# HarrisonKramer/optiland

Hardware: AMD Instinct MI355X
Metric: ray-surface intersections/s (higher is better)
Workload: dtype f32

## Files before the change

### include/optiland_hip.h

```cpp
#ifndef OPTILAND_HIP_H
#define OPTILAND_HIP_H

#include <stdint.h>

#ifdef __cplusplus
extern "C" {
#endif

#define OL_ABI_VERSION 11

#define OL_OK 0
#define OL_EINVAL (-1)
#define OL_EUNSUPPORTED (-2)
#define OL_EHIP (-3)
#define OL_ENOMEM (-4)

typedef int32_t ol_dtype;
enum { OL_F32 = 0, OL_F64 = 1 };

typedef enum ol_geom_kind {
  OL_GEOM_PLANE = 0,
  OL_GEOM_STANDARD = 1,
  OL_GEOM_EVEN_ASPHERE = 2,
  OL_GEOM_ZERNIKE = 3,
// ... 292 lines not shown
                   double Rp, double* psf_out, double* field_out, void* stream);

#define OL_MTF_MAX_CURVES 64
#define OL_MTF_MAX_BINS 8192
#define OL_MTF_NONFINITE 1
int ol_geometric_mtf(ol_dtype dt, int32_t n_curves, const void* const* coords,
                     const int64_t* lengths, int32_t num_points, const double* freq,
                     const double* scale, int32_t n_bins, double* mtf_out, int32_t* counts_out,
                     double* edges_minmax_out, int32_t* flags_out, void* stream);

#define OL_ZK_MAX_TERMS 120
#define OL_ZK_MAX_RADIAL 12
#define OL_ZK_MAX_M 32
#define OL_ZK_TOO_FEW 1
#define OL_ZK_RANK_DEFICIENT 2
#define OL_ZK_NONFINITE 4
#define OL_SMTF_MAX_FREQ 65535
int ol_zernike_fit(int32_t num_terms, const int32_t* term_i, const double* term_f, int64_t n,
                   const double* x, const double* y, const double* z, const double* intensity,
                   double* coeffs_out, int32_t* status_out, void* stream);
int ol_zernike_eval(int32_t num_terms, const int32_t* term_i, const double* term_f,
                    const double* coeffs, int64_t n, const double* x, const double* y,
                    double* out, void* stream);
int ol_sampled_mtf(int32_t num_terms, const int32_t* term_i, const double* term_f,
                   const double* coeffs, int64_t n, const double* x, const double* y,
                   const double* opd_waves, const double* p1, const double* intensity,
                   int32_t n_freq, const double* shifts, double* mtf_out, double* otf_out,
                   void* stream);

#define OL_TUNE_RAYS_PER_THREAD 0
#define OL_TUNE_COMPACT 1
#define OL_TUNE_FIT_GRID 2
#define OL_TUNE_RECORD_WG_CAP 3
int ol_set_tuning(int32_t knob, int32_t value);

const char* ol_last_error(void);
int32_t ol_abi_version(void);

#ifdef __cplusplus
}
#endif
#endif
```

### optiland_amd/_capi.py

```python

from __future__ import annotations

import ctypes as C
import os

from . import build as _build

_LIB = None


class HipExtensionError(RuntimeError):
    """The HIP shared library is missing / failed to load / returned an error."""


class SurfaceDesc(C.Structure):
    _fields_ = [
        ("geom_kind", C.c_int32),
        ("interaction", C.c_int32),
        ("aperture_kind", C.c_int32),
        ("coating_kind", C.c_int32),
        ("coeff_offset", C.c_int32),
        ("n_coeff", C.c_int32),
        ("max_iter", C.c_int32),
        ("flags", C.c_uint32),
# ... 85 lines not shown
    "ol_system_destroy",
    "ol_system_num_surfaces",
    "ol_trace",
    "ol_generate_rays",
    "ol_polarized_intensity",
    "ol_spot_moments",
    "ol_spot_max_r2",
    "ol_set_tuning",
    "ol_wavefront_opd",
    "ol_trace_spot",
    "ol_trace_ex",
    "ol_radial_energy",
    "ol_irradiance",
    "ol_trace_opd",
    "ol_pupil_fill",
    "ol_trace_generate",
    "ol_system_update",
    "ol_stream_fill",
    "ol_math_probe",
    "ol_pupil_points",
    "ol_wavefront_reference",
    "ol_trace_opd_dev",
    "ol_wavefront_fit",
    "ol_wavefront_opd_fitted",
    "ol_trace_spot_batch",
    "ol_newton_count",
    "ol_arena_alloc",
    "ol_arena_free",
    "ol_huygens_psf",
    "ol_geometric_mtf",
    "ol_zernike_fit",
    "ol_zernike_eval",
    "ol_sampled_mtf",
)

F32, F64 = 0, 1
TUNE_RAYS_PER_THREAD, TUNE_COMPACT, TUNE_FIT_GRID, TUNE_RECORD_WG_CAP = 0, 1, 2, 3
ABI_VERSION = 11
OPD_MOMENTS = 12
WAVEFRONT_REFERENCE_DOUBLES = 16
WAVEFRONT_FIT_WORKSPACE_DOUBLES = 32832
FIT_CENTROID, FIT_BEST_FIT = 0, 1
FIT_NO_VALID, FIT_TOO_FEW, FIT_NO_ALIVE, FIT_SINGULAR = 1, 2, 4, 8
FIT_STD_DDOF1, FIT_PISTON_SKIPS_NAN = 1, 2


def library_path() -> str:
    return os.environ.get("OPTILAND_HIP_LIBRARY", _build.library_path())


def load():
    global _LIB
    if _LIB is not None:
        return _LIB
    path = library_path()
    if not os.path.exists(path):
        raise HipExtensionError(
            f"HIP extension not built: {path} is missing. Run "
            "`python -c 'import __graft_entry__ as g; g.build()'` (needs hipcc). "
            "optiland_amd has no CPU fallback."
        )
    try:
        lib = C.CDLL(path)
    except OSError as exc:
        raise HipExtensionError(f"cannot load {path}: {exc}") from exc
    if hasattr(lib, "ol_hostmath_harness"):
        raise HipExtensionError(f"{path} is the host-math TEST harness, not the HIP extension")
    bind(lib, path)
    _LIB = lib
    return lib
# ... 49 lines not shown
        raise HipExtensionError(
            f"{path}: ABI version {have} != expected {ABI_VERSION}; rebuild"
        )
    lib.ol_wavefront_reference.restype = C.c_int
    lib.ol_wavefront_reference.argtypes = [vp, i32, vp, vp, vp, C.c_double, i32, i32, vp, vp, vp,
                                           vp]
    lib.ol_trace_opd_dev.restype = C.c_int
    lib.ol_trace_opd_dev.argtypes = [vp, i32, i64, vp, vp, vp, i32, vp, vp, C.POINTER(vp), vp,
                                     vp, vp]
    lib.ol_wavefront_fit.restype = C.c_int
    lib.ol_wavefront_fit.argtypes = [i32, vp, C.c_double, C.c_uint32, i32, i64, C.POINTER(vp), vp, vp,
                                     vp, vp, vp, vp]
    lib.ol_wavefront_opd_fitted.restype = C.c_int
    lib.ol_wavefront_opd_fitted.argtypes = [i64, C.POINTER(vp), vp, vp, vp, vp, C.POINTER(vp), vp]
    lib.ol_system_update.restype = C.c_int
    lib.ol_system_update.argtypes = [vp, vp, i32, vp, i32, vp, i32, vp]
    lib.ol_trace_generate.restype = C.c_int
    lib.ol_trace_generate.argtypes = [vp, C.c_int, i64, vp, vp, i32, vp, i64, C.POINTER(vp), vp,
                                      u32, vp, vp, vp]
    lib.ol_trace_spot_batch.restype = C.c_int
    lib.ol_trace_spot_batch.argtypes = [vp, C.c_int, i64, vp, vp, i32, vp, vp, i64, vp, vp, vp]
    lib.ol_newton_count.restype = C.c_int
    lib.ol_newton_count.argtypes = [vp, C.c_int, i64, C.POINTER(vp), i32, i32, i32, vp, i32, vp]
    lib.ol_arena_alloc.restype = C.c_int
    lib.ol_arena_alloc.argtypes = [i64, C.POINTER(vp)]
    lib.ol_arena_free.restype = C.c_int
    lib.ol_arena_free.argtypes = [vp]
    lib.ol_pupil_points.restype = C.c_int
    lib.ol_pupil_points.argtypes = [i32, i32, C.c_int, i64, vp, vp, vp, vp, vp]
    lib.ol_math_probe.restype = C.c_int
    lib.ol_math_probe.argtypes = [i32, C.c_int, i64, vp, vp, vp, vp]
    lib.ol_stream_fill.restype = C.c_int
    lib.ol_stream_fill.argtypes = [vp, i64, i32, i32, u32, vp]
    if hasattr(lib, "ol_huygens_psf"):
        lib.ol_huygens_psf.restype = C.c_int
        lib.ol_huygens_psf.argtypes = [i64, C.POINTER(vp), vp, i64, C.POINTER(vp), C.c_double,
                                       C.c_double, vp, vp, vp]
    if hasattr(lib, "ol_geometric_mtf"):
        lib.ol_geometric_mtf.restype = C.c_int
        lib.ol_geometric_mtf.argtypes = [C.c_int, i32, C.POINTER(vp), C.POINTER(i64), i32, vp, vp,
                                         i32, vp, vp, vp, vp, vp]
    if has_zernike_fit(lib):
        lib.ol_zernike_fit.restype = C.c_int
        lib.ol_zernike_fit.argtypes = [i32, vp, vp, i64, vp, vp, vp, vp, vp, vp, vp]
        lib.ol_zernike_eval.restype = C.c_int
        lib.ol_zernike_eval.argtypes = [i32, vp, vp, vp, i64, vp, vp, vp, vp]
        lib.ol_sampled_mtf.restype = C.c_int
        lib.ol_sampled_mtf.argtypes = [i32, vp, vp, vp, i64, vp, vp, vp, vp, vp, i32, vp, vp, vp,
                                       vp]
    return lib


ZK_MAX_TERMS, ZK_MAX_RADIAL, ZK_MAX_M, SMTF_MAX_FREQ = 120, 12, 32, 65535
ZK_TOO_FEW, ZK_RANK_DEFICIENT, ZK_NONFINITE = 1, 2, 4


def has_zernike_fit(lib) -> bool:
    return all(hasattr(lib, s) for s in ("ol_zernike_fit", "ol_zernike_eval", "ol_sampled_mtf"))


MTF_MAX_CURVES, MTF_MAX_BINS, MTF_NONFINITE = 64, 8192, 1


def has_geometric_mtf(lib) -> bool:
    return hasattr(lib, "ol_geometric_mtf")

# ... 12 lines not shown
```

### optiland_amd/csrc/capi.hip

```cpp
#include <hip/hip_runtime.h>

#include <algorithm>
#include <cmath>
#include <cstdarg>
#include <cstdio>
#include <cstdlib>
#include <cstring>
#include <map>
#include <new>
#include <string>
#include <type_traits>
#include <vector>

#include "../../include/optiland_hip.h"
#include "device_table.h"
#include "last_error.h"
#include "trace_launch.h"

namespace {
thread_local std::string g_err;
}

int ol::failf(int code, const char* fmt, ...) {
  char buf[512];
// ... 150 lines not shown
        }
      }
    }
  }
  for (int i = nmax; i >= 0; --i)
    for (int j = nmax - i; j >= 0; --j) out.push_back(S[i * W + j]);
  for (int i = nmax - 1; i >= 0; --i)
    for (int j = nmax - 1 - i; j >= 0; --j) {
      out.push_back((i + 1) * Q[(i + 1) * W + j]);
      out.push_back((j + 1) * Q[i * W + j + 1]);
    }
  *degree = nmax;
  return true;
}

struct HostSurf {
  int32_t geom, interaction, aperture_kind, coating_kind, coeff_off, n_coeff, max_iter;
  uint32_t flags;
  int32_t poly_cols, coeff_len, ap_off, ap_len;
  double cv, kp1, tol, inv_norm;
  double origin[3], rot[9], rel_off[3], rel_rot[9], ap[4], coat[2], axis[3], ret_cos, ret_sin;
  double radius, conic;
};

template <typename T>
struct DeviceTable {
  char* blob = nullptr;
  ol::DevSurfHot<T>* surf = nullptr;
  ol::DevSurfCold<T>* cold = nullptr;
  ol::DevOptics<T>* optics = nullptr;
  T* coeffs = nullptr;
  size_t n_surf = 0, n_opt = 0, coef_capacity = 0;
  size_t off_cold = 0, off_opt = 0, off_coef = 0;
};

inline size_t round256(size_t v) { return (v + 255u) & ~size_t(255u); }

struct Staged {
  std::vector<struct HostSurf> surf;
  std::vector<ol::DevOptics<double>> optics;
  std::vector<double> coeffs;
  std::vector<size_t> int_slots;
  std::vector<int32_t> interaction, coating, geom;
  std::vector<uint8_t> polygon, ref_newton, no_pair;
};

}

struct ol_system {
  int32_t n_surf = 0;
  int32_t n_wl = 0;
  int device = 0;
  DeviceTable<float> f32;
  DeviceTable<double> f64;
  std::vector<int32_t> interaction;
  std::vector<int32_t> coating;
  std::vector<int32_t> geom;
  std::vector<uint8_t> polygon;
  std::vector<uint8_t> ref_newton;
  std::vector<uint8_t> no_pair;
  bool consistent = true;
};

#define OL_CHECK_CONSISTENT(sys, who)                                                          \
  if (!(sys)->consistent)                                                                      \
    return failf(OL_EINVAL, who ": the system's tables are inconsistent after a failed "         \
                                "ol_system_update (destroy it and create a new one)")

namespace {

template <typename T>
int upload(const std::vector<HostSurf>& surf64,
           const std::vector<ol::DevOptics<double>>& opt64, const std::vector<double>& coef64,
           const std::vector<size_t>& int_slots, DeviceTable<T>& dst, bool in_place = false,
           hipStream_t stream = nullptr) {
  const size_t n_surf = surf64.size(), n_opt = opt64.size();
  const size_t n_coef = coef64.size() ? coef64.size() : 1;
  const size_t off_cold = round256(n_surf * sizeof(ol::DevSurfHot<T>));
  const size_t off_opt = off_cold + round256(n_surf * sizeof(ol::DevSurfCold<T>));
  const size_t off_coef = off_opt + round256(n_opt * sizeof(ol::DevOptics<T>));
  const size_t used = off_coef + n_coef * sizeof(T);
  std::vector<char> host(used, 0);
  auto* surf = reinterpret_cast<ol::DevSurfHot<T>*>(host.data());
  auto* cold = reinterpret_cast<ol::DevSurfCold<T>*>(host.data() + off_cold);
  auto* opt = reinterpret_cast<ol::DevOptics<T>*>(host.data() + off_opt);
  T* coef = reinterpret_cast<T*>(host.data() + off_coef);
  for (size_t i = 0; i < n_surf; ++i) {
    const auto& a = surf64[i];
    auto& b = surf[i];
    auto& c = cold[i];
    b.geom = a.geom; b.interaction = a.interaction; b.aperture_kind = a.aperture_kind;
    b.coating_kind = a.coating_kind; b.coeff_off = a.coeff_off; b.n_coeff = a.n_coeff;
    b.max_iter = a.max_iter; b.flags = a.flags;
    b.cv = (T)a.cv; b.kp1 = (T)a.kp1;
    c.poly_cols = a.poly_cols; c.coeff_len = a.coeff_len; c.ap_off = a.ap_off;
    c.ap_len = a.ap_len; c.tol = (T)a.tol; c.inv_norm = (T)a.inv_norm;
    for (int k = 0; k < 3; ++k) { b.origin[k] = (T)a.origin[k]; b.rel_off[k] = (T)a.rel_off[k]; }
    for (int k = 0; k < 9; ++k) { c.rot[k] = (T)a.rot[k]; c.rel_rot[k] = (T)a.rel_rot[k]; }
    for (int k = 0; k < 4; ++k) c.ap[k] = (T)a.ap[k];
    for (int k = 0; k < 2; ++k) c.coat[k] = (T)a.coat[k];
    for (int k = 0; k < 3; ++k) c.axis[k] = (T)a.axis[k];
    c.ret_cos = (T)a.ret_cos; c.ret_sin = (T)a.ret_sin;
    c.radius = (T)a.radius; c.conic = (T)a.conic;
  }
  for (size_t i = 0; i < n_opt; ++i) {
    opt[i].n1 = (T)opt64[i].n1; opt[i].n2 = (T)opt64[i].n2; opt[i].u = (T)opt64[i].u;
    opt[i].nn = (T)opt64[i].nn; opt[i].absorb = (T)opt64[i].absorb;
  }
  for (size_t i = 0; i < coef64.size(); ++i) coef[i] = (T)coef64[i];
  for (size_t i : int_slots) {
    using I = typename std::conditional<sizeof(T) == 4, int32_t, int64_t>::type;
    const I v = (I)coef64[i];
    std::memcpy(&coef[i], &v, sizeof(T));
  }

  if (in_place) {
    OL_HIP_CHECK(hipMemcpyAsync(dst.blob, host.data(), used, hipMemcpyHostToDevice, stream));
    return OL_OK;
  }
  dst.n_surf = n_surf;
  dst.n_opt = n_opt;
  dst.coef_capacity = n_coef + 64;
  dst.off_cold = off_cold; dst.off_opt = off_opt; dst.off_coef = off_coef;
  OL_HIP_CHECK(hipMalloc((void**)&dst.blob, off_coef + dst.coef_capacity * sizeof(T)));
  dst.surf = reinterpret_cast<ol::DevSurfHot<T>*>(dst.blob);
  dst.cold = reinterpret_cast<ol::DevSurfCold<T>*>(dst.blob + off_cold);
  dst.optics = reinterpret_cast<ol::DevOptics<T>*>(dst.blob + off_opt);
  dst.coeffs = reinterpret_cast<T*>(dst.blob + off_coef);
  OL_HIP_CHECK(hipMemcpy(dst.blob, host.data(), used, hipMemcpyHostToDevice));
  return OL_OK;
}

template <typename T>
void release(DeviceTable<T>& t) {
  if (t.blob) (void)hipFree(t.blob);
  t = DeviceTable<T>();
}

bool aligned16(const void* p) { return (reinterpret_cast<uintptr_t>(p) & 15u) == 0; }

int newton_family(const ol_system* sys, int32_t first, int32_t last) {
  bool any = false, polygon = false, all_zernike = true, all_even = true;
  for (int32_t s = first; s <= last; ++s)
    if (sys->ref_newton[s]) return ol::kNrReference;
  for (int32_t s = first; s <= last; ++s) {
    polygon = polygon || sys->polygon[s];
    const int g = sys->geom[s];
    if (g == OL_GEOM_PLANE || g == OL_GEOM_STANDARD) continue;
// ... 148 lines not shown
  if (a.in.hx == nullptr) ol::uniform_field_tangents<T>(rg, a.in);
  for (int k = 0; k < 8; ++k) a.rays[k] = rays_out ? static_cast<T*>(rays_out[k]) : nullptr;
  a.record = static_cast<T*>(record);
  a.prt = static_cast<T*>(prt);
  a.status = status;
  a.n = n;
  a.record_stride = record_stride;
  a.first = 0;
  a.last = sys->n_surf - 1;
  a.record_from = (extras && extras->record_first_surface > 0) ? extras->record_first_surface : 0;
  a.n_wl = sys->n_wl;
  a.wl = wl;
  a.flags = (flags & (ol::kTracePrtComplex | ol::kTraceFewWaves)) |
            (prt ? ol::kTracePrtIdentity : 0u) | (rays_out ? ol::kTraceWriteRays : 0u);
  if (extras && extras->updated_intensity && extras->update_intensity_state) {
    if (!prt)
      return failf(OL_EINVAL, "ol_trace_generate: the update_intensity epilogue needs a "
                              "polarised launch (prt)");
    const ol_polarization_state* ps = extras->update_intensity_state;
    ol::PolStateDev st{ps->is_polarized, ps->Ex, ps->Ey, ps->phase_x, ps->phase_y};
    a.pf = ol::PolFields<T>(st);
    a.i_updated = static_cast<T*>(extras->updated_intensity);
  }
  bool pair_ok = al && (reinterpret_cast<uintptr_t>(record) % 8 == 0) && record_stride % 2 == 0;
  if (rays_out)
    for (int k = 0; k < 8; ++k)
      pair_ok = pair_ok && reinterpret_cast<uintptr_t>(rays_out[k]) % 8 == 0;
  const int family = newton_family(sys, 0, sys->n_surf - 1);
  if (family == ol::kNrZernike) {
    for (int32_t s = 0; s < sys->n_surf; ++s) pair_ok = pair_ok && !sys->no_pair[s];
    pair_ok = pair_ok && prt && n % 2 == 0 && reinterpret_cast<uintptr_t>(prt) % 8 == 0 &&
              reinterpret_cast<uintptr_t>(a.i_updated) % 8 == 0;
  }
  hipError_t e = ol::launch_trace_generate<T>(a, family, pair_ok, stream);
  if (e != hipSuccess) return failf(OL_EHIP, "trace launch failed: %s", hipGetErrorString(e));
  return OL_OK;
}

template <typename T>
int do_trace_spot(const ol_system* sys, const DeviceTable<T>& tab, int64_t n,
                  const ol_raygen_params* p, const ol_raygen_inputs* in, double cx, double cy,
                  int32_t wl, void* const hits[3], double* out7, uint32_t* status,
                  hipStream_t stream) {
  ol::SpotArgs<T> a{};
  bool vec = true;
  if (int rc = convert_inputs<T>("ol_trace_spot", in, status, a.in, vec)) return rc;
  if (n == 0) return OL_OK;
  a.surf = tab.surf;
  a.cold = tab.cold;
  a.optics = tab.optics;
  a.coeffs = tab.coeffs;
  a.rg = raygen_dev(p);
  a.cx = cx;
  a.cy = cy;
  for (int k = 0; k < 3; ++k) {
    a.hits[k] = hits ? static_cast<T*>(hits[k]) : nullptr;
    vec = vec && aligned16(a.hits[k]);
  }
  a.out = out7;
  a.status = status;
  a.n = n;
  a.first = 0;
  a.last = sys->n_surf - 1;
  a.n_wl = sys->n_wl;
  a.wl = wl;
  a.tiles_per_block = 1;
// ... 132 lines not shown
      ol::launch_opd_trace<T>(a, vec, newton_family(sys, 0, sys->n_surf - 1), stream);
  if (e != hipSuccess) return failf(OL_EHIP, "opd launch failed: %s", hipGetErrorString(e));
  return OL_OK;
}

}

extern "C" {

const char* ol_last_error(void) { return g_err.c_str(); }
int32_t ol_abi_version(void) { return OL_ABI_VERSION; }

int ol_set_tuning(int32_t knob, int32_t value) {
  switch (knob) {
    case OL_TUNE_RAYS_PER_THREAD:
      if (value < 0 || value > 3)
        return failf(OL_EINVAL, "ol_set_tuning: rays per thread must be 0 (auto), 1, 2 (vector) "
                                "or 3 (fp32 pair)");
      ol::tuning().rays_per_thread = value;
      return OL_OK;
    case OL_TUNE_COMPACT:
      ol::tuning().compact = value ? 1 : 0;
      return OL_OK;
    case OL_TUNE_RECORD_WG_CAP:
      if (value < 0 || value > 8)
        return failf(OL_EINVAL, "ol_set_tuning: record workgroup cap 0 (default policy), "
                                "1 (never) or 2 ... 8");
      ol::tuning().record_wg_cap = value;
      return OL_OK;
    case OL_TUNE_FIT_GRID:
      if (value < 0 || value > ol::kFitMaxBlocks)
        return failf(OL_EINVAL, "ol_set_tuning: fit grid 0 (default) ... %d", ol::kFitMaxBlocks);
      ol::tuning().fit_grid = value;
      return OL_OK;
    default:
      return failf(OL_EINVAL, "ol_set_tuning: unknown knob %d", knob);
  }
}

namespace {
int stage_system(const char* who, const ol_surface_desc* surf, int32_t n_surf,
                 const double* coeffs, int32_t n_coeffs, const ol_surface_optics* optics,
                 int32_t n_wavelengths, Staged& st) {
  if (!surf || n_surf <= 0) return failf(OL_EINVAL, "%s: no surfaces", who);
  if (!optics || n_wavelengths <= 0) return failf(OL_EINVAL, "%s: no optics table", who);
  if (n_coeffs < 0 || (n_coeffs > 0 && !coeffs))
    return failf(OL_EINVAL, "%s: bad coefficient buffer", who);

  st.surf.assign(n_surf, HostSurf());
  std::vector<HostSurf>& dev = st.surf;
  std::vector<double>& dcoef = st.coeffs;
  std::vector<size_t>& int_slots = st.int_slots;
  int32_t prev_traced = -1;
  for (int32_t i = 0; i < n_surf; ++i) {
    const ol_surface_desc& s = surf[i];
    HostSurf& d = dev[i];
    std::memset(&d, 0, sizeof(d));
    if (s.geom_kind < OL_GEOM_PLANE || s.geom_kind > OL_GEOM_TOROIDAL)
      return failf(OL_EUNSUPPORTED, "surface %d: geometry kind %d", i, s.geom_kind);
    if (s.interaction < OL_INTERACT_RECORD_ONLY || s.interaction > OL_INTERACT_REFLECT)
      return failf(OL_EUNSUPPORTED, "surface %d: interaction %d", i, s.interaction);
    if (s.aperture_kind < OL_AP_NONE || s.aperture_kind > OL_AP_POLYGON)
      return failf(OL_EUNSUPPORTED, "surface %d: aperture kind %d", i, s.aperture_kind);
    if (s.coating_kind < OL_COAT_NONE || s.coating_kind > OL_COAT_RETARDER)
      return failf(OL_EUNSUPPORTED, "surface %d: coating kind %d", i, s.coating_kind);
    if (s.n_coeff < 0 || s.coeff_offset < 0)
// ... 241 lines not shown
                            n_wavelengths, st))
    return rc;
  OL_CHECK_CONSISTENT(sys, "ol_system_update");
  const size_t need = st.coeffs.size() ? st.coeffs.size() : 1;
  if (need > sys->f32.coef_capacity || need > sys->f64.coef_capacity)
    return failf(OL_EUNSUPPORTED, "ol_system_update: coefficient block of %zu values exceeds the "
                                  "allocated %zu", need, sys->f32.coef_capacity);
  {
    int cur = -1;
    if (hipGetDevice(&cur) != hipSuccess || cur != sys->device)
      return failf(OL_EINVAL, "ol_system_update: current HIP device %d is not the system's "
                              "device %d", cur, sys->device);
  }
  hipStream_t s = static_cast<hipStream_t>(stream);
  int rc = upload<double>(st.surf, st.optics, st.coeffs, st.int_slots, sys->f64, true, s);
  if (rc != OL_OK) return rc;
  sys->consistent = false;
  rc = upload<float>(st.surf, st.optics, st.coeffs, st.int_slots, sys->f32, true, s);
  if (rc != OL_OK) return rc;
  adopt_host_copies(sys, st);
  sys->consistent = true;
  return OL_OK;
}

void ol_system_destroy(ol_system* sys) {
  if (!sys) return;
  release(sys->f32);
  release(sys->f64);
  delete sys;
}

int32_t ol_system_num_surfaces(const ol_system* sys) { return sys ? sys->n_surf : 0; }

int ol_trace(const ol_system* sys, ol_dtype dt, int64_t n_rays, void* const rays[8],
             int32_t wavelength_index, void* record, int64_t record_stride, void* prt,
             int32_t first_surface, int32_t last_surface, uint32_t flags, uint32_t* status,
             void* stream) {
  return ol_trace_ex(sys, dt, n_rays, rays, wavelength_index, record, record_stride, prt,
                     first_surface, last_surface, flags, status, nullptr, stream);
}

int ol_trace_ex(const ol_system* sys, ol_dtype dt, int64_t n_rays, void* const rays[8],
                int32_t wavelength_index, void* record, int64_t record_stride, void* prt,
                int32_t first_surface, int32_t last_surface, uint32_t flags, uint32_t* status,
                const ol_trace_extras* extras, void* stream) {
  if (!sys) return failf(OL_EINVAL, "ol_trace: system is NULL");
  OL_CHECK_CONSISTENT(sys, "ol_trace");
  if (dt != OL_F32 && dt != OL_F64) return failf(OL_EINVAL, "ol_trace: bad dtype %d", (int)dt);
  if (n_rays < 0) return failf(OL_EINVAL, "ol_trace: negative ray count");
  if (first_surface < 0 || last_surface >= sys->n_surf || first_surface > last_surface)
    return failf(OL_EINVAL, "ol_trace: surface range [%d, %d] outside [0, %d)", first_surface,
                 last_surface, sys->n_surf);
  if (wavelength_index < 0 || wavelength_index >= sys->n_wl)
    return failf(OL_EINVAL, "ol_trace: wavelength index %d outside [0, %d)", wavelength_index,
                 sys->n_wl);
  if (n_rays == 0) return OL_OK;
  {
    int cur = -1;
    if (hipGetDevice(&cur) != hipSuccess || cur != sys->device)
      return failf(OL_EINVAL, "ol_trace: current HIP device %d is not the system's device %d",
                   cur, sys->device);
  }
  if (!rays) return failf(OL_EINVAL, "ol_trace: rays is NULL");
  for (int k = 0; k < 8; ++k)
    if (!rays[k]) return failf(OL_EINVAL, "ol_trace: rays[%d] is NULL", k);
  if (record && record_stride < n_rays)
// ... 663 lines not shown
```

### optiland_amd/csrc/device_table.h

```cpp
#pragma once
#include <stdint.h>

#ifdef OL_HOST_MATH
#define OL_DEV __host__ __device__ inline
#else
#define OL_DEV __device__ __forceinline__
#endif

#if defined(__HIP_DEVICE_COMPILE__)
#define OL_CONST_AS __attribute__((address_space(4)))
#else
#define OL_CONST_AS
#endif

namespace ol {
template <typename X>
using cptr = const OL_CONST_AS X*;

template <typename X>
OL_DEV cptr<X> as_const(const X* p) {
  return (cptr<X>)p;
}

template <typename P>
// ... 24 lines not shown
  kGeomStandard = 1,
  kGeomEvenAsphere = 2,
  kGeomZernike = 3,
  kGeomOddAsphere = 4,
  kGeomPolynomial = 5,
  kGeomChebyshev = 6,
  kGeomBiconic = 7,
  kGeomToroidal = 8,
  kGeomZernikeMono = 9
};
enum : int { kRecordOnly = 0, kRefract = 1, kReflect = 2 };
enum : int {
  kApNone = 0, kApRadial = 1, kApOffsetRadial = 2, kApRect = 3, kApElliptical = 4,
  kApComposite = 5, kApPolygon = 6, kApOpUnion = 10, kApOpIntersection = 11, kApOpDifference = 12
};
constexpr int kApTokenLen = 5;
enum : int {
  kCoatNone = 0, kCoatSimple = 1, kCoatFresnel = 2, kCoatPolarizer = 3, kCoatRetarder = 4
};

constexpr int kNrNone = 0;
constexpr int kNrGeneric = 1;
constexpr int kNrCompact = 2;
constexpr int kNrZernike = 3;
constexpr int kNrEvenAsphere = 4;
constexpr int kNrReference = 5;

constexpr uint32_t kPolNonUnitK = 0x1u;

constexpr uint32_t kSurfRotated = 0x1u;
constexpr uint32_t kSurfRelRotated = 0x2u;
constexpr uint32_t kSurfRadiusInf = 0x4u;
constexpr uint32_t kSurfReferenceRoot = 0x8u;

template <typename T>
struct alignas(16) DevSurfHot {
  int32_t geom;
  int32_t interaction;
  int32_t aperture_kind;
  int32_t coating_kind;
  uint32_t flags;
  int32_t coeff_off;
  int32_t n_coeff;
  int32_t max_iter;
  T cv;
  T kp1;
  T rel_off[3];
  T origin[3];
};

template <typename T>
struct DevSurfCold {
  int32_t poly_cols;
  int32_t coeff_len;
  int32_t ap_off;
  int32_t ap_len;
  T tol;
  T inv_norm;
  T rot[9];
  T rel_rot[9];
  T ap[4];
  T coat[2];
  T axis[3];
  T ret_cos, ret_sin;
  T radius, conic;
};
// ... 83 lines not shown
```

### optiland_amd/csrc/surface_math.h

```cpp
#pragma once
#include <hip/hip_runtime.h>
#include <math.h>
#include <stdint.h>

#include <type_traits>

#include "device_table.h"

namespace ol {
namespace hw {
#if defined(OL_HOST_MATH) && !defined(__HIP_DEVICE_COMPILE__)
OL_DEV float rcp(float x) { return 1.0f / x; }
OL_DEV float sqrt(float x) { return ::sqrtf(x); }
OL_DEV float rsq(float x) { return 1.0f / ::sqrtf(x); }
OL_DEV float exp(float x) { return ::expf(x); }
OL_DEV int float_bits(float x) { int i; __builtin_memcpy(&i, &x, 4); return i; }
OL_DEV long long double_bits(double x) { long long i; __builtin_memcpy(&i, &x, 8); return i; }
OL_DEV bool wave_any(bool v) { return v; }
OL_DEV int wave_max(int v) { return v; }
OL_DEV bool wave_leader() { return true; }
OL_DEV void atomic_max_i32(int32_t* p, int32_t v) { if (v > *p) *p = v; }
OL_DEV void atomic_or_i32(int32_t* p, int32_t v) { *p |= v; }
OL_DEV int32_t load_i32(const int32_t* p) { return *p; }
#else
// ... 2022 lines not shown
      r[k].x = m::fma(q[k].dt, r[k].L, q[k].xb);
      r[k].y = m::fma(q[k].dt, r[k].M, q[k].yb);
      r[k].z = m::fma(q[k].dt, r[k].N, q[k].zb);
      t[k] = t[k] + q[k].dt;
    }
    if (it == 0) {
      const DevSurf<T> s = h.surf();
      cptr<T> c = coeffs + s.coeff_off;
#pragma unroll
      for (int k = 0; k < RPT; ++k) {
        T sag;
        uint32_t st = 0;
        nr_eval<NR>(s, c, r[k].x, r[k].y, sag, q[k].gx, q[k].gy, st);
      }
    }
#pragma unroll
    for (int k = 0; k < RPT; ++k) {
      const T im = m::rsqrt(m::fma(q[k].gx, q[k].gx, m::fma(q[k].gy, q[k].gy, T(1))));
      nx[k] = q[k].gx * im;
      ny[k] = q[k].gy * im;
      nz[k] = -im;
    }
  } else {
#pragma unroll
    for (int k = 0; k < RPT; ++k) t[k] = nx[k] = ny[k] = nz[k] = m::splat(0);
  }
  {
    const DevSurf<T> s = h.surf();
    const DevOptics<T> o = h.optics();
    interact<V, RPT, POLK, NR != 0>(s, o, coeffs, t, nx, ny, nz, r, P, prt_fresh, pol_flags);
  }
}

template <typename V, int RPT, int POLK, int NR, bool SHARE = false>
OL_DEV void surface_step(const DevSurf<typename Math<V>::scalar>& s,
                         const DevOptics<typename Math<V>::scalar>& o,
                         cptr<typename Math<V>::scalar> coeffs, bool from_global,
                         Ray<V> (&r)[RPT],
                         Prt<typename PrtLane<V, POLK>::type, POLK> (&P)[POLK ? RPT : 1],
                         uint32_t& status, bool& prt_fresh, const NrRefCtl* ref = nullptr,
                         uint32_t pol_flags = 0) {
  const SurfLoaded<typename Math<V>::scalar> h{s, o};
  surface_step<V, RPT, POLK, NR, SHARE>(h, coeffs, from_global, r, P, status, prt_fresh, ref,
                                        pol_flags);
}

template <typename V>
OL_DEV Ray<V> to_global(const DevSurf<typename Math<V>::scalar>& s,
                                            const Ray<V>& r) {
  using T = typename Math<V>::scalar;
  Ray<V> g = r;
  if (s.flags & kSurfRotated) {
    cptr<T> R = s.cold->rot;
    g.x = R[0] * r.x + R[3] * r.y + R[6] * r.z;
    g.y = R[1] * r.x + R[4] * r.y + R[7] * r.z;
    g.z = R[2] * r.x + R[5] * r.y + R[8] * r.z;
    g.L = R[0] * r.L + R[3] * r.M + R[6] * r.N;
    g.M = R[1] * r.L + R[4] * r.M + R[7] * r.N;
    g.N = R[2] * r.L + R[5] * r.M + R[8] * r.N;
  }
  g.x += s.origin[0];
  g.y += s.origin[1];
  g.z += s.origin[2];
  return g;
}

}
```

### optiland_amd/csrc/trace_kernel.hip

```cpp
#include <hip/hip_runtime.h>
#include <stdint.h>
#include <math.h>
#include <stdlib.h>

#include <type_traits>

#include "device_table.h"
#include "raygen_device.h"
#include "wavefront_device.h"
#include "epilogue_device.h"
#include "trace_launch.h"

#ifndef OL_TABLE_IN_LDS
#define OL_TABLE_IN_LDS 0
#endif
#ifndef OL_NR_PREFETCH
#define OL_NR_PREFETCH 0
#endif
#ifndef OL_PREFETCH_F64
#define OL_PREFETCH_F64 1
#endif
#ifndef OL_FUSED_NR_PREFETCH
#define OL_FUSED_NR_PREFETCH 1
#endif
// ... 279 lines not shown
                        as_const(optics) + (s * n_wl + wl)};
}
#ifndef OL_POLNR_WAVES_F64
#define OL_POLNR_WAVES_F64 0
#endif
#ifndef OL_LEAN_F64_WAVES
#define OL_LEAN_F64_WAVES 0
#endif
#ifndef OL_POLZ_PAIR_WAVES
#define OL_POLZ_PAIR_WAVES 0
#endif
template <typename T, int RPT, int POLK, int NR, bool GEN = false>
struct WavesPerEu {
  static constexpr int value =
      (OL_POLZ_PAIR_WAVES > 0 && sizeof(T) == 4 && RPT == 2 && POLK == 1 && NR == kNrZernike)
          ? OL_POLZ_PAIR_WAVES
      : (OL_POLNR_WAVES > 0 && sizeof(T) == 4 && RPT == 1 && POLK == 1 && NR != 0 &&
       NR != kNrReference && !(GEN && NR == 1))
          ? OL_POLNR_WAVES
          : ((OL_POLNR_WAVES_F64 > 0 && sizeof(T) == 8 && RPT == 1 && POLK == 1 && NR != 0)
                 ? OL_POLNR_WAVES_F64
                 : ((OL_LEAN_F64_WAVES > 0 && sizeof(T) == 8 && RPT == 1 && POLK == 0 && NR == 0)
                        ? OL_LEAN_F64_WAVES
                        : 1));
};

template <typename T, int RPT = 1>
__device__ __forceinline__ T (*epi_launch_slots())[kTraceBlock * RPT] {
  __shared__ T slots[4][kTraceBlock * RPT];
  return slots;
}

template <typename T, int RPT, bool RECORD, int POLK, int NR, bool SPOT, int GEN = 0,
          bool EPI = false>
__global__ __launch_bounds__(kTraceBlock)
__attribute__((amdgpu_waves_per_eu(WavesPerEu<T, RPT, POLK, NR, GEN != 0 || EPI>::value))) void trace_kernel(
    const DevSurfHot<T>* __restrict__ surf_tab, const DevSurfCold<T>* __restrict__ cold_tab,
    const DevOptics<T>* __restrict__ optics_tab, const T* __restrict__ coeff_tab,
    TraceArgs<T> a) {
#if OL_TABLE_IN_LDS
  constexpr int kMaxLdsSurf = 64;
  __shared__ DevSurfHot<T> lds_hot[kMaxLdsSurf];
  __shared__ DevOptics<T> lds_opt[kMaxLdsSurf];
  {
    const int ns = a.last - a.first + 1;
    constexpr int HW = sizeof(DevSurfHot<T>) / 4, OW = sizeof(DevOptics<T>) / 4;
    const uint32_t* gh = reinterpret_cast<const uint32_t*>(surf_tab + a.first);
    uint32_t* lh = reinterpret_cast<uint32_t*>(lds_hot);
    for (int i = threadIdx.x; i < ns * HW; i += kTraceBlock) lh[i] = gh[i];
    uint32_t* lo = reinterpret_cast<uint32_t*>(lds_opt);
    for (int i = threadIdx.x; i < ns * OW; i += kTraceBlock) {
      const int sidx = i / OW, w = i % OW;
      lo[i] = reinterpret_cast<const uint32_t*>(optics_tab + (a.first + sidx) * a.n_wl + a.wl)[w];
    }
    __syncthreads();
  }
#endif
  using RayIndex = RayIndexT<(OL_SADDR != 0) && POLK != 0>;
  RayIndex base{(int64_t)blockIdx.x * (kTraceBlock * RPT), (uint32_t)threadIdx.x * RPT};
  const bool live = base.full() < a.n;
  if constexpr (!SPOT) {
    if (!live) return;
  } else if (RPT == 1 && !live) {
    base.lane = (uint32_t)(a.n - 1 - base.tile);
  }
  const int64_t left = a.n - base.full();
  const int cnt = RPT == 1 ? 1 : (left >= RPT ? RPT : (left > 0 ? (int)left : 0));
// ... 137 lines not shown
#pragma unroll
          for (int e = 0; e < NPRT; ++e)
#pragma unroll
            for (int k = 0; k < RPT; ++k)
              pin[e][k] = k < cnt ? base.at(a.prt + (int64_t)e * a.n)[k] : T(0);
        }
      }
    }
#pragma unroll
    for (int k = 0; k < RPT; ++k) {
      Ray<T> o;
      o.x = in[0][k]; o.y = in[1][k]; o.z = in[2][k];
      o.L = in[3][k]; o.M = in[4][k]; o.N = in[5][k];
      o.i = in[6][k]; o.opd = in[7][k];
      LP::put(r, k, o);
      if constexpr (POLK != 0) {
        const bool ident = (a.flags & kTracePrtIdentity) != 0;
#pragma unroll
        for (int e = 0; e < NPRT; ++e)
          LP::pset(P, k, e, ident ? ((e == 0 || e == 4 || e == 8) ? T(1) : T(0)) : pin[e][k]);
      }
    }
  }

  bool is_global = true;
  bool prt_fresh = POLK != 0 && (GEN != 0 || (a.flags & kTracePrtIdentity) != 0);
  constexpr bool kFetch = fetch_level<T, NR, false, POLK>() >= 2;
  constexpr bool kFetchArgs = fetch_level<T, NR, false, POLK>() >= 1;
  const cptr<T> coeffs_c = as_const(coeff_tab);
  constexpr bool kShareRcp = !RECORD && RPT > 1;
  DevSurf<T> last_traced;
  last_traced.cold = as_const(cold_tab);
  int last_idx = a.first;
  auto to_global_now = [&](Ray<V> (&gv)[NV]) {
    if constexpr (kFetch) {
      const DevSurf<T> lt = fetched_surface<T, TraceArgs<T>>(last_idx).surf();
#pragma unroll
      for (int j = 0; j < NV; ++j) gv[j] = is_global ? r[j] : to_global<V>(lt, r[j]);
    } else {
#pragma unroll
      for (int j = 0; j < NV; ++j) gv[j] = is_global ? r[j] : to_global<V>(last_traced, r[j]);
    }
  };
#if OL_TABLE_IN_LDS
  DevSurfHot<T> cur = lds_hot[0];
#else
  constexpr bool kPrefetch = (OL_NR_PREFETCH || NR == 0) && (OL_PREFETCH_F64 || sizeof(T) == 4);
  DevSurfHot<T> cur;
  if constexpr (!kFetch) cur = surf_tab[a.first];
#endif
  const int first = a.first, last = a.last;
  const int rec_from = a.record_from > first ? a.record_from : first;
  for (int s = first; s <= last; ++s) {
    uint32_t polf = 0;
    if constexpr (POLK != 0 && GEN == 0) {
      uint32_t fl;
      if constexpr (kFetchArgs) fl = kernargs<T, TraceArgs<T>>()->a.flags;
      else fl = a.flags;
      polf = (fl & kTraceNonUnitK) ? kPolNonUnitK : 0u;
    }
    if constexpr (kFetch) {
      const SurfFetched<T> h = fetched_surface<T, TraceArgs<T>>(s);
      if (refresh(h.hot)->interaction != kRecordOnly) {
        if constexpr (NR == kNrReference) {
          const auto ka = kernargs<T, TraceArgs<T>>();
          const NrRefCtl ctl{ka->a.nr_iters, s, ka->a.n_surf, ka->a.nr_count_at};
          surface_step<V, NV, POLK, NR, kShareRcp>(h, refresh(coeffs_c), is_global, r, P, status,
                                                 prt_fresh, &ctl, polf);
        } else {
          surface_step<V, NV, POLK, NR, kShareRcp>(h, refresh(coeffs_c), is_global, r, P, status,
                                                 prt_fresh, nullptr, polf);
        }
        is_global = false;
        last_idx = s;
      }
    } else {
      DevSurf<T> S;
#if OL_TABLE_IN_LDS
      static_cast<DevSurfHot<T>&>(S) = cur;
      if (s < a.last) cur = lds_hot[s + 1 - a.first];
#else
      if constexpr (kPrefetch) {
        static_cast<DevSurfHot<T>&>(S) = cur;
        if (s < a.last) cur = surf_tab[s + 1];
      } else {
// ... 164 lines not shown
    {
      PolFields<T> f;
#pragma unroll
      for (int k = 0; k < 2; ++k) {
        f.ar[k] = ka->a.pf.ar[k]; f.ai[k] = ka->a.pf.ai[k];
        f.br[k] = ka->a.pf.br[k]; f.bi[k] = ka->a.pf.bi[k];
      }
      f.nf = ka->a.pf.nf;
      T (*epi_launch)[kTraceBlock * RPT] = epi_launch_slots<T, RPT>();
      T upd_k[RPT];
#pragma unroll
      for (int k = 0; k < RPT; ++k) {
        T Pm[9], Qm[9];
#pragma unroll
        for (int e = 0; e < 9; ++e) {
          Pm[e] = LP::pget(P, k, e);
          Qm[e] = POLK == 2 ? LP::pget(P, k, POLK == 2 ? 9 + e : e) : T(0);
        }
        const int slot = threadIdx.x * RPT + k;
        const T L0 = epi_launch[0][slot], M0 = epi_launch[1][slot], N0 = epi_launch[2][slot],
                i0 = epi_launch[3][slot];
        uint32_t st_k = 0;
        upd_k[k] = pol_intensity_one<T, POLK == 2>(f, L0, M0, N0, Pm, Qm, i0, st_k);
        if (k < cnt) status |= st_k;
      }
      if constexpr (RPT == 1) base.at(upd)[0] = upd_k[0];
      else store_plane<T, RPT>(upd, base, cnt, upd_k);
    }
  }
  if (status && late.status) atomicOr(late.status, status);
}

template <typename T>
static unsigned record_lds(const TraceArgs<T>& a, bool lean, bool generating) {
  if (a.record == nullptr) return 0;
  int cap = tuning().record_wg_cap;
  if (cap == 0)
    cap = !lean ? 1 : sizeof(T) == 8 ? 3 : !(a.flags & kTraceFewWaves) ? 1 : generating ? 2 : 3;
  if (cap < 2) return 0;
  const unsigned want = 160u * 1024u / (unsigned)cap - 1024u;
  return want > 63u * 1024u ? 63u * 1024u : want;
}

template <typename T, int RPT, int NR>
static hipError_t launch_nr(const TraceArgs<T>& a, hipStream_t stream) {
  const int64_t threads = (a.n + RPT - 1) / RPT;
  const int64_t blocks = (threads + kTraceBlock - 1) / kTraceBlock;
  if (blocks == 0) return hipSuccess;
  if (blocks > 0x7fffffffLL) return hipErrorInvalidValue;
  dim3 grid((unsigned)blocks), block(kTraceBlock);
  const bool rec = a.record != nullptr;
  const int polk = a.prt == nullptr ? 0 : ((a.flags & kTracePrtComplex) ? 2 : 1);
#define OL_LAUNCH_S(R, P, S)                                                                 \
  hipLaunchKernelGGL((trace_kernel<T, RPT, R, P, NR, S>), grid, block,                        \
                     record_lds(a, NR == 0 && P == 0, false), stream, a.surf, a.cold,         \
                     a.optics, a.coeffs, a)
#define OL_LAUNCH(R, P) OL_LAUNCH_S(R, P, false)
  if (a.spot != nullptr) {
    if (polk != 0 || NR == kNrReference) return hipErrorInvalidValue;
    if constexpr (NR != kNrReference) {
      if (rec) OL_LAUNCH_S(true, 0, true); else OL_LAUNCH_S(false, 0, true);
    }
    return hipGetLastError();
  }
  if (polk == 2) {
    if constexpr (RPT == 1) {
      if (rec) OL_LAUNCH(true, 2); else OL_LAUNCH(false, 2);
    } else {
      return hipErrorInvalidValue;
    }
  } else if (rec && polk == 1) OL_LAUNCH(true, 1);
  else if (rec) OL_LAUNCH(true, 0);
  else if (polk == 1) OL_LAUNCH(false, 1);
  else OL_LAUNCH(false, 0);
// ... 14 lines not shown
    }
    if (nr == kNrReference) return launch_nr<T, 1, kNrReference>(a, stream);
  }
  return launch_nr<T, RPT, 1>(a, stream);
}

template <typename T>
static hipError_t launch_pair(const TraceArgs<T>& a, hipStream_t stream) {
  const int64_t threads = (a.n + 1) / 2;
  const int64_t blocks = (threads + kTraceBlock - 1) / kTraceBlock;
  if (blocks == 0) return hipSuccess;
  if (blocks > 0x7fffffffLL) return hipErrorInvalidValue;
  dim3 grid((unsigned)blocks), block(kTraceBlock);
  if (a.record != nullptr)
    hipLaunchKernelGGL((trace_kernel<T, 2, true, 0, 0, false>), grid, block,
                       record_lds(a, true, false), stream, a.surf, a.cold, a.optics, a.coeffs,
                       a);
  else
    hipLaunchKernelGGL((trace_kernel<T, 2, false, 0, 0, false>), grid, block, 0, stream, a.surf,
                       a.cold, a.optics, a.coeffs, a);
  return hipGetLastError();
}

#ifndef OL_GEN_PAIR
#define OL_GEN_PAIR 1
#endif
template <typename T>
static hipError_t launch_gen_pair(const TraceArgs<T>& a, hipStream_t stream) {
  const int64_t threads = (a.n + 1) / 2;
  const int64_t blocks = (threads + kTraceBlock - 1) / kTraceBlock;
  if (blocks == 0) return hipSuccess;
  if (blocks > 0x7fffffffLL) return hipErrorInvalidValue;
  const dim3 grid((unsigned)blocks), block(kTraceBlock);
  if (a.spot != nullptr)
    hipLaunchKernelGGL((trace_kernel<T, 2, true, 0, 0, true, kGenUniform, false>), grid, block,
                       record_lds(a, true, true), stream, a.surf, a.cold, a.optics, a.coeffs, a);
  else
    hipLaunchKernelGGL((trace_kernel<T, 2, true, 0, 0, false, kGenUniform, false>), grid, block,
                       record_lds(a, true, true), stream, a.surf, a.cold, a.optics, a.coeffs, a);
  return hipGetLastError();
}

template <typename T, int NR>
static hipError_t launch_gen_nr(const TraceArgs<T>& a, bool pair_ok, hipStream_t stream) {
  if constexpr (sizeof(T) == 4 && NR == 0) {
    const int want = tuning().rays_per_thread;
    if (pair_ok && a.prt == nullptr && a.in.hx == nullptr && a.rgc.apod_kind == 0 &&
        (want == 3 || (want == 0 && OL_GEN_PAIR)))
      return launch_gen_pair<T>(a, stream);
  }
  if constexpr (sizeof(T) == 4 && NR == kNrZernike) {
    const int want = tuning().rays_per_thread;
    if (pair_ok && a.prt != nullptr && !(a.flags & kTracePrtComplex) && a.spot == nullptr &&
        a.n % 2 == 0 && reinterpret_cast<uintptr_t>(a.prt) % 8 == 0 &&
        reinterpret_cast<uintptr_t>(a.i_updated) % 8 == 0 &&
        (want == 3 || (want == 0 && OL_POLZ_PAIR))) {
      const int64_t threads = (a.n + 1) / 2;
      const int64_t blocks2 = (threads + kTraceBlock - 1) / kTraceBlock;
      if (blocks2 == 0) return hipSuccess;
      if (blocks2 > 0x7fffffffLL) return hipErrorInvalidValue;
      const dim3 grid2((unsigned)blocks2), block2(kTraceBlock);
      if (a.i_updated != nullptr)
        hipLaunchKernelGGL((trace_kernel<T, 2, true, 1, NR, false, kGenUniform, true>), grid2,
                           block2, 0, stream, a.surf, a.cold, a.optics, a.coeffs, a);
      else
        hipLaunchKernelGGL((trace_kernel<T, 2, true, 1, NR, false, kGenUniform, false>), grid2,
// ... 671 lines not shown
```

### optiland_amd/csrc/trace_launch.h

```cpp
#pragma once
#include <hip/hip_runtime.h>
#include <math.h>
#include <stdint.h>

#include "device_table.h"

namespace ol {

#ifndef OL_TRACE_BLOCK
#define OL_TRACE_BLOCK 256
#endif
constexpr int kTraceBlock = OL_TRACE_BLOCK;
constexpr uint32_t kTraceWriteRays = 0x1u;
constexpr uint32_t kTraceCompact = 0x2u;
constexpr uint32_t kTracePrtComplex = 0x4u;
constexpr uint32_t kTracePrtIdentity = 0x8u;
constexpr uint32_t kTraceFewWaves = 0x10u;
constexpr uint32_t kTraceNonUnitK = 0x20u;
constexpr uint32_t kTraceRow0IsInput = 0x100u;

constexpr int kGenUniform = 1;
constexpr int kGenFieldPlanes = 2;
constexpr int kGenApod = 4;

#ifndef OL_POLZ_PAIR
#define OL_POLZ_PAIR 1
#endif

struct Tuning {
  int rays_per_thread = 0;
  int compact = 0;
  int fit_grid = 0;
  int record_wg_cap = 0;
};
Tuning& tuning();

struct RaygenDev {
  int32_t object_infinite;
  int32_t field_kind;
  double EPL, EPD, max_field, offset, z_first, tele_dz;
  double apod_a, apod_b;
  int32_t apod_kind;
};

#if defined(__HIPCC__)
#define OL_HD __host__ __device__
#else
#define OL_HD
#endif
template <typename T>
struct RaygenConsts {
  T EPL, EPD, maxf, off_epl, z_inf, z_fin, epl_z, tele_dz, apod_a, apod_b;
  int32_t apod_kind;
  int32_t infinite, height, linear, telecentric;
  RaygenConsts() = default;
  OL_HD explicit RaygenConsts(const RaygenDev& p)
      : EPL((T)p.EPL), EPD((T)p.EPD), maxf((T)p.max_field), off_epl((T)(p.offset + p.EPL)),
        z_inf((T)(p.z_first - p.offset)), z_fin((T)p.z_first), epl_z((T)(p.EPL - p.z_first)),
        tele_dz((T)p.tele_dz), apod_a((T)p.apod_a), apod_b((T)p.apod_b),
        apod_kind(p.apod_kind), infinite(p.object_infinite != 0),
        height(p.field_kind == 1 || (p.field_kind == 2 && p.object_infinite == 0)),
        linear(p.field_kind != 0), telecentric(p.tele_dz > 0.0) {}
};

constexpr uint32_t kRaygenCheckField = 0x1u;
constexpr uint32_t kRaygenCheckPupil = 0x2u;
constexpr uint32_t kRaygenPrescalePupil = 0x4u;
constexpr uint32_t kSpotPolarizedOk = 0x8u;
// ... 278 lines not shown
```

Baseline: 207.2 billion.

## Add coaxial fast path for fp32 generating trace of plain spherical systems

```diff
diff --git a/include/optiland_hip.h b/include/optiland_hip.h
--- a/include/optiland_hip.h
+++ b/include/optiland_hip.h
@@ -348,7 +348,12 @@
 #define OL_TUNE_COMPACT 1
 #define OL_TUNE_FIT_GRID 2
 #define OL_TUNE_RECORD_WG_CAP 3
+#define OL_TUNE_COAXIAL 4
 int ol_set_tuning(int32_t knob, int32_t value);
+
+int32_t ol_system_coaxial(const ol_system* sys);
+uint32_t ol_record_lds_request(ol_dtype dt, int32_t lean, int32_t generating, int32_t coaxial,
+                               uint32_t flags);
 
 const char* ol_last_error(void);
 int32_t ol_abi_version(void);
diff --git a/optiland_amd/_capi.py b/optiland_amd/_capi.py
--- a/optiland_amd/_capi.py
+++ b/optiland_amd/_capi.py
@@ -141,10 +141,13 @@
     "ol_zernike_fit",
     "ol_zernike_eval",
     "ol_sampled_mtf",
+    "ol_system_coaxial",
+    "ol_record_lds_request",
 )
 
 F32, F64 = 0, 1
 TUNE_RAYS_PER_THREAD, TUNE_COMPACT, TUNE_FIT_GRID, TUNE_RECORD_WG_CAP = 0, 1, 2, 3
+TUNE_COAXIAL = 4
 ABI_VERSION = 11
 OPD_MOMENTS = 12
 WAVEFRONT_REFERENCE_DOUBLES = 16
@@ -260,6 +263,11 @@
     lib.ol_math_probe.argtypes = [i32, C.c_int, i64, vp, vp, vp, vp]
     lib.ol_stream_fill.restype = C.c_int
     lib.ol_stream_fill.argtypes = [vp, i64, i32, i32, u32, vp]
+    if hasattr(lib, "ol_system_coaxial"):
+        lib.ol_system_coaxial.restype = i32
+        lib.ol_system_coaxial.argtypes = [vp]
+        lib.ol_record_lds_request.restype = u32
+        lib.ol_record_lds_request.argtypes = [C.c_int, i32, i32, i32, u32]
     if hasattr(lib, "ol_huygens_psf"):
         lib.ol_huygens_psf.restype = C.c_int
         lib.ol_huygens_psf.argtypes = [i64, C.POINTER(vp), vp, i64, C.POINTER(vp), C.c_double,
diff --git a/optiland_amd/csrc/capi.hip b/optiland_amd/csrc/capi.hip
--- a/optiland_amd/csrc/capi.hip
+++ b/optiland_amd/csrc/capi.hip
@@ -206,6 +206,7 @@
   T* coeffs = nullptr;
   size_t n_surf = 0, n_opt = 0, coef_capacity = 0;
   size_t off_cold = 0, off_opt = 0, off_coef = 0;
+  bool coaxial = false;
 };
 
 inline size_t round256(size_t v) { return (v + 255u) & ~size_t(255u); }
@@ -242,6 +243,26 @@
                                 "ol_system_update (destroy it and create a new one)")
 
 namespace {
+
+template <typename T>
+bool coaxial_eligible(const ol::DevSurfHot<T>* surf, size_t n_surf) {
+  auto plus_zero = [](T v) { return v == T(0) && !std::signbit(v); };
+  bool entered = false;
+  for (size_t i = 0; i < n_surf; ++i) {
+    const auto& h = surf[i];
+    if (h.interaction == ol::kRecordOnly) continue;
+    if (h.interaction != ol::kRefract) return false;
+    if (h.geom != ol::kGeomPlane && h.geom != ol::kGeomStandard) return false;
+    if (h.geom == ol::kGeomStandard && h.kp1 != T(1)) return false;
+    if (h.flags & ~(ol::kSurfRadiusInf | ol::kSurfCoaxial)) return false;
+    if (h.coating_kind != ol::kCoatNone) return false;
+    if (h.aperture_kind != ol::kApNone && h.aperture_kind != ol::kApRadial) return false;
+    if (!plus_zero(h.origin[0]) || !plus_zero(h.origin[1])) return false;
+    if (entered && (!plus_zero(h.rel_off[0]) || !plus_zero(h.rel_off[1]))) return false;
+    entered = true;
+  }
+  return entered;
+}
 
 template <typename T>
 int upload(const std::vector<HostSurf>& surf64,
@@ -288,6 +309,9 @@
     std::memcpy(&coef[i], &v, sizeof(T));
   }
 
+  dst.coaxial = coaxial_eligible<T>(surf, n_surf);
+  if (dst.coaxial && sizeof(T) == 4)
+    for (size_t i = 0; i < n_surf; ++i) surf[i].flags |= ol::kSurfCoaxial;
   if (in_place) {
     OL_HIP_CHECK(hipMemcpyAsync(dst.blob, host.data(), used, hipMemcpyHostToDevice, stream));
     return OL_OK;
@@ -502,6 +526,7 @@
     pair_ok = pair_ok && prt && n % 2 == 0 && reinterpret_cast<uintptr_t>(prt) % 8 == 0 &&
               reinterpret_cast<uintptr_t>(a.i_updated) % 8 == 0;
   }
+  if (sizeof(T) == 4 && tab.coaxial && ol::coaxial_knob()) a.flags |= ol::kTraceCoaxial;
   hipError_t e = ol::launch_trace_generate<T>(a, family, pair_ok, stream);
   if (e != hipSuccess) return failf(OL_EHIP, "trace launch failed: %s", hipGetErrorString(e));
   return OL_OK;
@@ -700,6 +725,9 @@
       if (value < 0 || value > ol::kFitMaxBlocks)
         return failf(OL_EINVAL, "ol_set_tuning: fit grid 0 (default) ... %d", ol::kFitMaxBlocks);
       ol::tuning().fit_grid = value;
+      return OL_OK;
+    case OL_TUNE_COAXIAL:
+      ol::coaxial_knob() = value ? 1 : 0;
       return OL_OK;
     default:
       return failf(OL_EINVAL, "ol_set_tuning: unknown knob %d", knob);
@@ -1007,6 +1035,16 @@
 
 int32_t ol_system_num_surfaces(const ol_system* sys) { return sys ? sys->n_surf : 0; }
 
+int32_t ol_system_coaxial(const ol_system* sys) {
+  return sys && sys->consistent && sys->f32.coaxial ? 1 : 0;
+}
+
+uint32_t ol_record_lds_request(ol_dtype dt, int32_t lean, int32_t generating, int32_t coaxial,
+                               uint32_t flags) {
+  return ol::record_lds_request(true, dt == OL_F64, flags, lean != 0, generating != 0,
+                                coaxial != 0, ol::tuning().record_wg_cap);
+}
+
 int ol_trace(const ol_system* sys, ol_dtype dt, int64_t n_rays, void* const rays[8],
              int32_t wavelength_index, void* record, int64_t record_stride, void* prt,
              int32_t first_surface, int32_t last_surface, uint32_t flags, uint32_t* status,
diff --git a/optiland_amd/csrc/device_table.h b/optiland_amd/csrc/device_table.h
--- a/optiland_amd/csrc/device_table.h
+++ b/optiland_amd/csrc/device_table.h
@@ -80,6 +80,12 @@
 constexpr uint32_t kSurfRelRotated = 0x2u;
 constexpr uint32_t kSurfRadiusInf = 0x4u;
 constexpr uint32_t kSurfReferenceRoot = 0x8u;
+constexpr uint32_t kSurfCoaxial = 0x10u;
+
+inline int& coaxial_knob() {
+  static int v = 1;
+  return v;
+}
 
 template <typename T>
 struct alignas(16) DevSurfHot {
diff --git a/optiland_amd/csrc/surface_math.h b/optiland_amd/csrc/surface_math.h
--- a/optiland_amd/csrc/surface_math.h
+++ b/optiland_amd/csrc/surface_math.h
@@ -2078,6 +2078,11 @@
   }
 }
 
+template <typename V>
+OL_DEV void surface_step_coaxial(const DevSurfHot<float>& s, cptr<DevSurfCold<float>> cold,
+                                 const DevOptics<float>& o, float dz, Ray<V> (&r)[1],
+                                 uint32_t& status);
+
 template <typename V, int RPT, int POLK, int NR, bool SHARE = false>
 OL_DEV void surface_step(const DevSurf<typename Math<V>::scalar>& s,
                          const DevOptics<typename Math<V>::scalar>& o,
@@ -2086,9 +2091,50 @@
                          Prt<typename PrtLane<V, POLK>::type, POLK> (&P)[POLK ? RPT : 1],
                          uint32_t& status, bool& prt_fresh, const NrRefCtl* ref = nullptr,
                          uint32_t pol_flags = 0) {
+#if defined(OL_HOST_MATH) && !defined(__HIP_DEVICE_COMPILE__)
+  if constexpr (std::is_same<V, f32x2>::value && RPT == 1 && POLK == 0 && NR == 0 && !SHARE) {
+    if ((s.flags & kSurfCoaxial) && coaxial_knob()) {
+      surface_step_coaxial<V>(s, s.cold, o, from_global ? -s.origin[2] : s.rel_off[2], r, status);
+      return;
+    }
+  }
+#endif
   const SurfLoaded<typename Math<V>::scalar> h{s, o};
   surface_step<V, RPT, POLK, NR, SHARE>(h, coeffs, from_global, r, P, status, prt_fresh, ref,
                                         pol_flags);
+}
+
+template <typename V>
+OL_DEV void surface_step_coaxial(const DevSurfHot<float>& s, cptr<DevSurfCold<float>> cold,
+                                 const DevOptics<float>& o, float dz, Ray<V> (&r)[1],
+                                 uint32_t& status) {
+  static_assert(std::is_same<V, f32x2>::value, "the coaxial arm: the fp32 packed pair");
+  DevSurf<float> S;
+  S.geom = s.geom == kGeomPlane ? kGeomPlane : kGeomStandard;
+  S.interaction = kRefract;
+  S.aperture_kind = s.aperture_kind != kApNone ? kApRadial : kApNone;
+  S.coating_kind = kCoatNone;
+  S.flags = s.flags & kSurfRadiusInf;
+  S.coeff_off = 0;
+  S.n_coeff = 0;
+  S.max_iter = 0;
+  S.cv = s.cv;
+  S.kp1 = 1.0f;
+  S.rel_off[0] = S.rel_off[1] = -0.0f;
+  S.rel_off[2] = dz;
+  S.origin[0] = S.origin[1] = S.origin[2] = 0.0f;
+  S.cold = cold;
+  DevOptics<float> O;
+  O.n1 = o.n1;
+  O.n2 = o.n2;
+  O.u = o.u;
+  O.nn = o.nn;
+  O.absorb = o.absorb;
+  Prt<float, 0> P[1];
+  bool prt_fresh = false;
+  surface_step<V, 1, 0, 0, false>(S, O, cptr<float>(nullptr), false, r, P, status, prt_fresh);
+  r[0].x = r[0].x + Math<V>::splat(0.0f);
+  r[0].y = r[0].y + Math<V>::splat(0.0f);
 }
 
 template <typename V>
diff --git a/optiland_amd/csrc/trace_kernel.hip b/optiland_amd/csrc/trace_kernel.hip
--- a/optiland_amd/csrc/trace_kernel.hip
+++ b/optiland_amd/csrc/trace_kernel.hip
@@ -335,7 +335,7 @@
 }
 
 template <typename T, int RPT, bool RECORD, int POLK, int NR, bool SPOT, int GEN = 0,
-          bool EPI = false>
+          bool EPI = false, bool COAX = false>
 __global__ __launch_bounds__(kTraceBlock)
 __attribute__((amdgpu_waves_per_eu(WavesPerEu<T, RPT, POLK, NR, GEN != 0 || EPI>::value))) void trace_kernel(
     const DevSurfHot<T>* __restrict__ surf_tab, const DevSurfCold<T>* __restrict__ cold_tab,
@@ -539,8 +539,15 @@
   DevSurf<T> last_traced;
   last_traced.cold = as_const(cold_tab);
   int last_idx = a.first;
+  T coax_oz = T(-0.0);
   auto to_global_now = [&](Ray<V> (&gv)[NV]) {
-    if constexpr (kFetch) {
+    if constexpr (COAX) {
+#pragma unroll
+      for (int j = 0; j < NV; ++j) {
+        gv[j] = r[j];
+        gv[j].z = r[j].z + coax_oz;
+      }
+    } else if constexpr (kFetch) {
       const DevSurf<T> lt = fetched_surface<T, TraceArgs<T>>(last_idx).surf();
 #pragma unroll
       for (int j = 0; j < NV; ++j) gv[j] = is_global ? r[j] : to_global<V>(lt, r[j]);
@@ -558,6 +565,48 @@
 #endif
   const int first = a.first, last = a.last;
   const int rec_from = a.record_from > first ? a.record_from : first;
+  if constexpr (COAX) {
+    static_assert(sizeof(T) == 4 && RPT == 2 && NV == 1 && RECORD && POLK == 0 && NR == 0 &&
+                      GEN == kGenUniform && !EPI && !kFetch && !OL_TABLE_IN_LDS,
+                  "the coaxial arm: the lean fp32 generating pair");
+    T* plane = a.record + base.tile;
+    const int64_t stride = a.record_stride;
+    const bool ragged = __any(cnt != RPT) != 0;
+    const RayIndexT<true> lane_only{0, base.lane};
+    for (int s = first; s <= last; ++s) {
+      const DevSurfHot<T> S = cur;
+      if (s < last) cur = surf_tab[s + 1];
+      if (S.interaction != kRecordOnly) {
+        const DevOptics<T> O = optics_tab[s * a.n_wl + a.wl];
+        const T dz = is_global ? -S.origin[2] : S.rel_off[2];
+        surface_step_coaxial<V>(S, as_const(cold_tab) + s, O, dz, r, status);
+        is_global = false;
+        coax_oz = S.origin[2];
+      }
+      if (s >= rec_from) {
+        if (s == first && (a.flags & kTraceRow0IsInput)) {
+          plane += 8 * stride;
+        } else {
+          const V f[8] = {r[0].x, r[0].y, r[0].z + coax_oz, r[0].L, r[0].M, r[0].N, r[0].i,
+                          r[0].opd};
+          if (!ragged) {
+#pragma unroll
+            for (int q = 0; q < 8; ++q) {
+              __builtin_nontemporal_store(f[q], reinterpret_cast<V*>(plane + base.lane));
+              plane += stride;
+            }
+          } else {
+#pragma unroll
+            for (int q = 0; q < 8; ++q) {
+              const T tmp[RPT] = {f[q].x, f[q].y};
+              store_plane<T, RPT>(plane, lane_only, cnt, tmp);
+              plane += stride;
+            }
+          }
+        }
+      }
+    }
+  } else
   for (int s = first; s <= last; ++s) {
     uint32_t polf = 0;
     if constexpr (POLK != 0 && GEN == 0) {
@@ -788,14 +837,10 @@
 }
 
 template <typename T>
-static unsigned record_lds(const TraceArgs<T>& a, bool lean, bool generating) {
-  if (a.record == nullptr) return 0;
-  int cap = tuning().record_wg_cap;
-  if (cap == 0)
-    cap = !lean ? 1 : sizeof(T) == 8 ? 3 : !(a.flags & kTraceFewWaves) ? 1 : generating ? 2 : 3;
-  if (cap < 2) return 0;
-  const unsigned want = 160u * 1024u / (unsigned)cap - 1024u;
-  return want > 63u * 1024u ? 63u * 1024u : want;
+static unsigned record_lds(const TraceArgs<T>& a, bool lean, bool generating,
+                           bool coaxial = false) {
+  return record_lds_request(a.record != nullptr, sizeof(T) == 8, a.flags, lean, generating, coaxial,
+                            tuning().record_wg_cap);
 }
 
 template <typename T, int RPT, int NR>
@@ -876,6 +921,17 @@
   if (blocks == 0) return hipSuccess;
   if (blocks > 0x7fffffffLL) return hipErrorInvalidValue;
   const dim3 grid((unsigned)blocks), block(kTraceBlock);
+  if (a.flags & kTraceCoaxial) {
+    if (a.spot != nullptr)
+      hipLaunchKernelGGL((trace_kernel<T, 2, true, 0, 0, true, kGenUniform, false, true>), grid,
+                         block, record_lds(a, true, true, true), stream, a.surf, a.cold, a.optics,
+                         a.coeffs, a);
+    else
+      hipLaunchKernelGGL((trace_kernel<T, 2, true, 0, 0, false, kGenUniform, false, true>), grid,
+                         block, record_lds(a, true, true, true), stream, a.surf, a.cold, a.optics,
+                         a.coeffs, a);
+    return hipGetLastError();
+  }
   if (a.spot != nullptr)
     hipLaunchKernelGGL((trace_kernel<T, 2, true, 0, 0, true, kGenUniform, false>), grid, block,
                        record_lds(a, true, true), stream, a.surf, a.cold, a.optics, a.coeffs, a);
diff --git a/optiland_amd/csrc/trace_launch.h b/optiland_amd/csrc/trace_launch.h
--- a/optiland_amd/csrc/trace_launch.h
+++ b/optiland_amd/csrc/trace_launch.h
@@ -18,6 +18,7 @@
 constexpr uint32_t kTraceFewWaves = 0x10u;
 constexpr uint32_t kTraceNonUnitK = 0x20u;
 constexpr uint32_t kTraceRow0IsInput = 0x100u;
+constexpr uint32_t kTraceCoaxial = 0x200u;
 
 constexpr int kGenUniform = 1;
 constexpr int kGenFieldPlanes = 2;
@@ -34,6 +35,22 @@
   int record_wg_cap = 0;
 };
 Tuning& tuning();
+
+#ifndef OL_COAXIAL_WG_CAP
+#define OL_COAXIAL_WG_CAP 1
+#endif
+inline unsigned record_lds_request(bool recording, bool fp64, uint32_t flags, bool lean,
+                                   bool generating, bool coaxial, int tuned) {
+  if (!recording) return 0;
+  int cap = tuned;
+  if (cap == 0) {
+    cap = !lean ? 1 : fp64 ? 3 : !(flags & kTraceFewWaves) ? 1 : generating ? 2 : 3;
+    if (lean && !fp64 && generating && coaxial && OL_COAXIAL_WG_CAP > 1) cap = OL_COAXIAL_WG_CAP;
+  }
+  if (cap < 2) return 0;
+  const unsigned want = 160u * 1024u / (unsigned)cap - 1024u;
+  return want > 63u * 1024u ? 63u * 1024u : want;
+}
 
 struct RaygenDev {
   int32_t object_infinite;
```

After: 196.6 billion. 0.949x the previous value.
